# ZephirFXEC/HNanoSolver

Measured on AMD Instinct MI355X. Metric: solver substeps/sec (advect + 50 red-black SOR iterations + project) at N active voxels, higher is better.
Workload: dtype f32

## Files before the change

hnanosolver_amd/csrc/hns_sorblock.hip:

```cpp
#include "hns_device.hpp"
#include "hns_flags.hpp"

namespace hns {


template <int LB, int K>
struct SbGeo {
	static constexpr int H = 2 * K;
	static constexpr int T = 8 * LB + 2 * H;
	static constexpr int C = LB + 2;
	static constexpr int HALF = T / 2;
	static constexpr int ROWS = T * T / 2;
	static constexpr int TC = T - 2;
	static constexpr int HC = TC / 2;
	static constexpr int CROWS = TC * HC;
	static constexpr int RIM = 2 * TC;
	static constexpr int SEC = (CROWS + 63) / 64 * 64;
	static constexpr int NT = 2 * SEC;
	static constexpr int NQ = (HALF + 3) / 4;
	static constexpr int HS4 = 3;
	static constexpr int NCH = T / 4;
	static constexpr int REC = LB == 1 ? 28 : 64;
	static_assert(H % 4 == 0 && H <= 8, "rows must start on a 16-byte piece and stay within the neighbouring leaf");
	static_assert(NQ <= HS4 && NT <= 1024 && RIM <= CROWS, "tile too large");
};

constexpr float kInv6 = 0.166666667f;

template <bool MASKED>
__device__ __forceinline__ float sb_update(float xp, float xm, float yp, float ym, float zp, float zm, float d, float X, float omega, unsigned ok) {
	const float pGS = ((xp + xm + yp + ym + zp + zm) - d) * kInv6;
	const float cand = X + omega * (pGS - X);
	return MASKED ? __uint_as_float(__float_as_uint(cand) & ok) : cand;
}

template <int HALF, int C>
struct SbRow {
	float R[HALF], B[HALF];
	float dR[HALF], dB[HALF];
	unsigned ok[C];
};

template <int LB, int K>
struct SbLds {
	using G = SbGeo<LB, K>;
	static constexpr int NB = G::ROWS * G::HS4, NR = (G::ROWS - 2 * G::HALF) * G::HS4;
	float4 a[2 * (NB + NR)];
	__device__ __forceinline__ float4* arr(int par, int colour) { return a + par * (NB + NR) + (colour ? 0 : NB - G::HALF * G::HS4); }
};

template <int LB, int K, int S, int NS, bool PAR, bool MASKED, class Row>
__device__ __forceinline__ void sb_sweep(Row& r, SbLds<LB, K>& L, const int i, const int b, const int dist, const float omega) {
	using G = SbGeo<LB, K>;
	constexpr int H = G::H, HALF = G::HALF, HS4 = G::HS4;
	constexpr bool red = (S & 1) != 0;
	float(&X)[HALF] = red ? r.R : r.B;
	const float(&Y)[HALF] = red ? r.B : r.R;
	const float(&dX)[HALF] = red ? r.dR : r.dB;
	const float4* LY = L.arr(PAR ? 0 : 1, red ? 1 : 0);
	float4* LX = L.arr(PAR ? 1 : 0, red ? 0 : 1);
	constexpr bool up = red ? PAR : !PAR;
	constexpr int qlo = (S / 2) / 4, qhi = (HALF - S / 2 + 3) / 4;
	constexpr int jlo = 4 * qlo, jhi = 4 * qhi < HALF ? 4 * qhi : HALF;
	if (dist >= S) {
		const float4* pxp = LY + (i + HALF) * HS4;
		const float4* pxm = LY + (i - HALF) * HS4;
		const float4* pyp = LY + (i + b) * HS4;
		const float4* pym = LY + (i + b - 1) * HS4;
		float4 nx[4] = {pxp[qlo], pxm[qlo], pyp[qlo], pym[qlo]};
#pragma unroll
		for (int q = qlo; q < qhi; ++q) {
			const float4 xp4 = nx[0], xm4 = nx[1], yp4 = nx[2], ym4 = nx[3];
			if (q + 1 < qhi) nx[0] = pxp[q + 1], nx[1] = pxm[q + 1], nx[2] = pyp[q + 1], nx[3] = pym[q + 1];
			__builtin_amdgcn_sched_barrier(0);
			const float xp[4] = {xp4.x, xp4.y, xp4.z, xp4.w}, xm[4] = {xm4.x, xm4.y, xm4.z, xm4.w};
			const float yp[4] = {yp4.x, yp4.y, yp4.z, yp4.w}, ym[4] = {ym4.x, ym4.y, ym4.z, ym4.w};
#pragma unroll
			for (int e = 0; e < 4; ++e) {
				const int j = 4 * q + e;
				if (j < jlo || j >= jhi) continue;
				const float below = j > 0 ? Y[j > 0 ? j - 1 : 0] : 0.0f, above = j + 1 < HALF ? Y[j + 1 < HALF ? j + 1 : 0] : 0.0f;
				const float zm = up ? Y[j] : below, zp = up ? above : Y[j];
				const int cz = (2 * j - H + 8) >> 3;
				X[j] = sb_update<MASKED>(xp[e], xm[e], yp[e], ym[e], zp, zm, dX[j], X[j], omega, r.ok[cz]);
			}
			__builtin_amdgcn_sched_barrier(0);
		}
		if (S < NS) {
#pragma unroll
			for (int q = qlo; q < qhi; ++q) {
				const int j = 4 * q;
				LX[i * HS4 + q] = make_float4(X[j], j + 1 < HALF ? X[j + 1 < HALF ? j + 1 : 0] : 0.0f, j + 2 < HALF ? X[j + 2 < HALF ? j + 2 : 0] : 0.0f,
				                              j + 3 < HALF ? X[j + 3 < HALF ? j + 3 : 0] : 0.0f);
			}
		}
	}
	if (S < NS) __syncthreads();
}

template <int LB, int K, int S, int NS, bool PAR, bool MASKED>
struct SbSweeps {
	template <class Row>
	static __device__ __forceinline__ void run(Row& r, SbLds<LB, K>& L, const int i, const int b, const int dist, const float omega) {
		sb_sweep<LB, K, S, NS, PAR, MASKED>(r, L, i, b, dist, omega);
		if constexpr (S < NS) SbSweeps<LB, K, S + 1, NS, PAR, MASKED>::run(r, L, i, b, dist, omega);
	}
};

template <int LB, int K, bool ZERO, bool PAR, int NS>
__device__ __forceinline__ void sb_body(SbLds<LB, K>& L, const int t, const int* __restrict__ recs, const float* __restrict__ div, const float* __restrict__ p_in,
                                        float* __restrict__ p_out, const unsigned field_bytes, const float dx2, const float omega) {
	using G = SbGeo<LB, K>;
	constexpr int H = G::H, T = G::T, C = G::C, HALF = G::HALF, NQ = G::NQ, NCH = G::NCH, HS4 = G::HS4;
	const bool valid = t < G::CROWS;
	const int xq = valid ? t / G::HC : 0;
	const int x = 1 + xq, y = valid ? 1 + 2 * (t - xq * G::HC) + ((x + 1 + (PAR ? 1 : 0)) & 1) : 1;
	const int b = y & 1;
	const int i = x * HALF + (y >> 1);
	const int dist = valid ? min(min(x, T - 1 - x), min(y, T - 1 - y)) : -1;
	const int cx = (x - H + 8) >> 3, cy = (y - H + 8) >> 3;
	const unsigned row_bytes = (unsigned)(((((x - H) & 7) << 3) | ((y - H) & 7)) * 32);
	const int* __restrict__ rec = recs + (size_t)blockIdx.x * G::REC + (LB == 1 ? 1 : 0) + (cx * C + cy) * C;
	unsigned base[C];
	SbRow<HALF, C> r;
#pragma unroll
	for (int cz = 0; cz < C; ++cz) {
		const int id = valid ? rec[cz] : -1;
		r.ok[cz] = id >= 0 ? 0xFFFFFFFFu : 0u;
		base[cz] = (unsigned)id * 2048u + row_bytes;
	}
	const v4i rp = field_rsrc(p_in, field_bytes), rd = field_rsrc(div, field_bytes), ro = field_rsrc(p_out, field_bytes);
	v4f32 pc[NCH], dc[NCH];
#pragma unroll
	for (int j = 0; j < NCH; ++j) {
		const int cz = (4 * j - H + 8) >> 3, zl = (4 * j - H) & 7;
		const unsigned off = base[cz] + (unsigned)(zl * 4);
		dc[j] = hns_buffer_load_v4f32(rd, (int)off, 0, 0);
		if (ZERO) pc[j] = v4f32{0.0f, 0.0f, 0.0f, 0.0f};
		else pc[j] = hns_buffer_load_v4f32(rp, (int)off, 0, 0);
	}
	if (t < G::RIM) {
		const int side = t / G::HC, m = t - side * G::HC;
		const int along = 2 * m + (((side & 1) != 0) == PAR ? 2 : 1);
		const int rx = side == 0 ? 0 : (side == 1 ? T - 1 : along), ry = side == 2 ? 0 : (side == 3 ? T - 1 : along);
		const int rcx = (rx - H + 8) >> 3, rcy = (ry - H + 8) >> 3;
		const unsigned rrow = (unsigned)(((((rx - H) & 7) << 3) | ((ry - H) & 7)) * 32);
		const int* __restrict__ rrec = recs + (size_t)blockIdx.x * G::REC + (LB == 1 ? 1 : 0) + (rcx * C + rcy) * C;
		unsigned rbase[C];
#pragma unroll
		for (int cz = 0; cz < C; ++cz) rbase[cz] = (unsigned)rrec[cz] * 2048u + rrow;
		v4f32 rc[NCH];
#pragma unroll
		for (int j = 0; j < NCH; ++j) rc[j] = ZERO ? v4f32{0.0f, 0.0f, 0.0f, 0.0f} : hns_buffer_load_v4f32(rp, (int)(rbase[(4 * j - H + 8) >> 3] + (unsigned)(((4 * j - H) & 7) * 4)), 0, 0);
		float4* LR = L.arr(PAR ? 1 : 0, 0) + (rx * HALF + (ry >> 1)) * HS4;
		float4* LK = L.arr(PAR ? 1 : 0, 1) + (rx * HALF + (ry >> 1)) * HS4;
		float rr[HALF + 4], rb[HALF + 4];
#pragma unroll
		for (int j = 0; j < NCH; ++j) {
			rr[2 * j] = PAR ? rc[j].y : rc[j].x, rb[2 * j] = PAR ? rc[j].x : rc[j].y;
			rr[2 * j + 1] = PAR ? rc[j].w : rc[j].z, rb[2 * j + 1] = PAR ? rc[j].z : rc[j].w;
		}
#pragma unroll
		for (int q = 0; q < NQ; ++q) {
			if (side >= 2) LR[q] = make_float4(rr[4 * q], rr[4 * q + 1], 4 * q + 2 < HALF ? rr[4 * q + 2] : 0.0f, 4 * q + 3 < HALF ? rr[4 * q + 3] : 0.0f);
			LK[q] = make_float4(rb[4 * q], rb[4 * q + 1], 4 * q + 2 < HALF ? rb[4 * q + 2] : 0.0f, 4 * q + 3 < HALF ? rb[4 * q + 3] : 0.0f);
		}
	}
#pragma unroll
	for (int j = 0; j < NCH; ++j) {
		r.R[2 * j] = PAR ? pc[j].y : pc[j].x, r.B[2 * j] = PAR ? pc[j].x : pc[j].y;
		r.R[2 * j + 1] = PAR ? pc[j].w : pc[j].z, r.B[2 * j + 1] = PAR ? pc[j].z : pc[j].w;
		const float d0 = dc[j].x * dx2, d1 = dc[j].y * dx2, d2 = dc[j].z * dx2, d3 = dc[j].w * dx2;
		r.dR[2 * j] = PAR ? d1 : d0, r.dB[2 * j] = PAR ? d0 : d1;
		r.dR[2 * j + 1] = PAR ? d3 : d2, r.dB[2 * j + 1] = PAR ? d2 : d3;
	}
	if (valid) {
		float4* LR = L.arr(PAR ? 1 : 0, 0) + i * HS4;
		float4* LK = L.arr(PAR ? 1 : 0, 1) + i * HS4;
#pragma unroll
		for (int q = 0; q < NQ; ++q) {
			const int j = 4 * q;
			LR[q] = make_float4(r.R[j], r.R[j + 1], j + 2 < HALF ? r.R[j + 2 < HALF ? j + 2 : 0] : 0.0f, j + 3 < HALF ? r.R[j + 3 < HALF ? j + 3 : 0] : 0.0f);
			LK[q] = make_float4(r.B[j], r.B[j + 1], j + 2 < HALF ? r.B[j + 2 < HALF ? j + 2 : 0] : 0.0f, j + 3 < HALF ? r.B[j + 3 < HALF ? j + 3 : 0] : 0.0f);
		}
	}
	bool mine = true;
#pragma unroll
	for (int cz = 0; cz < C; ++cz) mine = mine && (r.ok[cz] != 0u || !valid);
	const bool all_present = __syncthreads_and(mine) != 0;
	if (all_present)
		SbSweeps<LB, K, 1, NS, PAR, false>::run(r, L, i, b, dist, omega);
	else
		SbSweeps<LB, K, 1, NS, PAR, true>::run(r, L, i, b, dist, omega);
	if (dist >= H) {
#pragma unroll
		for (int j = H / 4; j < NCH - H / 4; ++j) {
			const int cz = (4 * j - H + 8) >> 3, zl = (4 * j - H) & 7;
			v4f32 v;
			v.x = PAR ? r.B[2 * j] : r.R[2 * j], v.y = PAR ? r.R[2 * j] : r.B[2 * j];
			v.z = PAR ? r.B[2 * j + 1] : r.R[2 * j + 1], v.w = PAR ? r.R[2 * j + 1] : r.B[2 * j + 1];
			hns_buffer_store_v4f32(v, ro, (int)(base[cz] + (unsigned)(zl * 4)), 0, 0);
		}
	}
}

template <int C, int HALF>
struct SbLeanRow {
	float dR[HALF], dB[HALF];
	unsigned ok[C];
};

__device__ __forceinline__ void chain_store_piece(const PhaseMirror& m, int leaf, bool mine, int row, int half, v4f32 v) {
	const int e1 = m.first[leaf + 1];
	for (int e = m.first[leaf]; e < e1; ++e) {
		const int2 t = m.entry[e];
		if (!mine) continue;
		const unsigned bits = m.mask ? (m.mask[(size_t)e * 64 + row] >> (4 * half)) & 0xFu : 0xFu;
		float* r = chain_out(m, t.x, 0) + (size_t)t.y * 512 + row * 8 + 4 * half;
		if (bits == 0xFu) {
			store_through(r, chain_v4f{v.x, v.y, v.z, v.w});
		} else if (bits) {
			const float f[4] = {v.x, v.y, v.z, v.w};
#pragma unroll
			for (int z = 0; z < 4; ++z)
				if (bits >> z & 1) store_through(r + z, f[z]);
		}
	}
}

__device__ __forceinline__ void chain_store_piece(const PackMirror& m, int leaf, bool mine, int row, int half, v4f32 v) {
	const int e1 = m.first[leaf + 1];
	for (int e = m.first[leaf]; e < e1; ++e) {
		const int2 t = m.entry[e];
		if (!mine) continue;
		const unsigned byte = m.mask[(size_t)e * 64 + row];
		const unsigned bits = (byte >> (4 * half)) & 0xFu;
		if (!bits) continue;
		float* q = m.msg[t.x] + (size_t)t.y + m.row_pre[(size_t)e * 64 + row] + __popc(byte & ((1u << (4 * half)) - 1u));
		const float f[4] = {v.x, v.y, v.z, v.w};
		int c = 0;
#pragma unroll
		for (int z = 0; z < 4; ++z)
			if (bits >> z & 1) q[c++] = f[z];
	}
}

struct SbLdsXY {
	using G = SbGeo<2, 2>;
	static constexpr int T = G::T, TC = G::TC, HS4 = G::HS4;
	static constexpr int NB = (T * TC + 2 * T) * HS4, NR = TC * TC * HS4;
	float4 a[NB + NR];
	__device__ __forceinline__ float4* black() { return a; }
	__device__ __forceinline__ float4* red() { return a + NB; }
	static __device__ __forceinline__ int brow(int x, int y) { return x * TC + y - 1; }
	static __device__ __forceinline__ int brim(int x, int y) { return T * TC + 2 * x + (y != 0); }
};
static_assert(sizeof(SbLdsXY) == 50880, "the XY form must fit three workgroups per CU (160 KB of LDS)");

template <int S, int NS, bool MASKED, class Row>
__device__ __forceinline__ void sb_sweep_xy(Row& r, SbLdsXY& L, const int bi, const int ypb, const int ymb, const int par, const int dist, const float omega) {
	using G = SbGeo<2, 2>;
	constexpr int H = G::H, HALF = G::HALF, HS4 = G::HS4, NQ = G::NQ, TC = G::TC;
	constexpr bool red = (S & 1) != 0;
	const float(&dX)[HALF] = red ? r.dR : r.dB;
	const bool up = red ? par != 0 : par == 0;
	constexpr int jlo = S / 2, jhi = (G::T - 1 - S) / 2 + 1;
	constexpr int qlo = jlo / 4, qhi = (jhi + 3) / 4;
	if (dist >= S) {
		v4f32* LXo4 = reinterpret_cast<v4f32*>((red ? L.red() + (bi - TC) * HS4 : L.black() + bi * HS4));
		const v4f32* LYo4 = reinterpret_cast<const v4f32*>((red ? L.black() + bi * HS4 : L.red() + (bi - TC) * HS4));
		const float4* LY = red ? L.black() : L.red() - TC * HS4;
		float Y[HALF];
#pragma unroll
		for (int q = 0; q < NQ; ++q) {
			const v4f32 y4 = LYo4[q];
			Y[4 * q] = y4.x, Y[4 * q + 1] = y4.y, Y[4 * q + 2] = y4.z, Y[4 * q + 3] = y4.w;
		}
		const v4f32* pxp = reinterpret_cast<const v4f32*>(LY + (bi + TC) * HS4);
		const v4f32* pxm = reinterpret_cast<const v4f32*>(LY + (bi - TC) * HS4);
		const v4f32* pyp = reinterpret_cast<const v4f32*>(LY + (red ? ypb : bi + 1) * HS4);
		const v4f32* pym = reinterpret_cast<const v4f32*>(LY + (red ? ymb : bi - 1) * HS4);
#pragma unroll
		for (int q = qlo; q < qhi; ++q) {
			v4f32 x4 = LXo4[q], xp4 = pxp[q], xm4 = pxm[q], yp4 = pyp[q], ym4 = pym[q];
			if (4 * q < jlo || 4 * q + 4 > jhi) {
				asm volatile("" : "+v"(x4));
				asm volatile("" : "+v"(xp4));
				asm volatile("" : "+v"(xm4));
				asm volatile("" : "+v"(yp4));
				asm volatile("" : "+v"(ym4));
			}
			float X[4] = {x4.x, x4.y, x4.z, x4.w};
			const float xp[4] = {xp4.x, xp4.y, xp4.z, xp4.w}, xm[4] = {xm4.x, xm4.y, xm4.z, xm4.w}, yp[4] = {yp4.x, yp4.y, yp4.z, yp4.w}, ym[4] = {ym4.x, ym4.y, ym4.z, ym4.w};
#pragma unroll
			for (int e = 0; e < 4; ++e) {
				const int j = 4 * q + e;
				if (j < jlo || j >= jhi) continue;
				const float below = j > 0 ? Y[j > 0 ? j - 1 : 0] : 0.0f, above = j + 1 < HALF ? Y[j + 1 < HALF ? j + 1 : 0] : 0.0f;
				const float zm = up ? Y[j] : below, zp = up ? above : Y[j];
				const int cz = (2 * j - H + 8) >> 3;
				X[e] = sb_update<MASKED>(xp[e], xm[e], yp[e], ym[e], zp, zm, dX[j], X[e], omega, r.ok[cz]);
			}
			v4f32 o4 = v4f32{X[0], X[1], X[2], X[3]};
			if (4 * q < jlo || 4 * q + 4 > jhi) asm volatile("" : "+v"(o4));
			LXo4[q] = o4;
			__builtin_amdgcn_sched_barrier(0);
		}
	}
	if (S < NS) __syncthreads();
}

template <int S, int NS, bool MASKED>
struct SbSweepsXY {
	template <class Row>
	static __device__ __forceinline__ void run(Row& r, SbLdsXY& L, const int bi, const int ypb, const int ymb, const int par, const int dist, const float omega) {
		sb_sweep_xy<S, NS, MASKED>(r, L, bi, ypb, ymb, par, dist, omega);
		if constexpr (S < NS) SbSweepsXY<S + 1, NS, MASKED>::run(r, L, bi, ypb, ymb, par, dist, omega);
	}
};

template <bool ZERO, class M = NoMirror, int NS = 4>
__global__ __attribute__((amdgpu_waves_per_eu(6, 8))) __launch_bounds__((SbGeo<2, 2>::NT)) void k_rbgs_block_xy(const int* __restrict__ recs, const int* __restrict__ any_absent, const float* __restrict__ div, const float* __restrict__ p_in,
                                                                                                                float* __restrict__ p_out, const unsigned field_bytes, const float dx2, const float omega, const M m = M{}) {
	using G = SbGeo<2, 2>;
	constexpr int H = G::H, T = G::T, C = G::C, HALF = G::HALF, NCH = G::NCH, HS4 = G::HS4, TC = G::TC;
	__shared__ SbLdsXY L;
	__shared__ int s_rec[64];
	const int t = threadIdx.x;
	const bool valid = t < TC * TC;
	const int xq = valid ? t / TC : 0;
	const int x = 1 + xq, y = valid ? 1 + t - xq * TC : 1;
	const int par = (x + y) & 1;
	const int bi = SbLdsXY::brow(x, y);
	const int ypb = y == T - 2 ? SbLdsXY::brim(x, T - 1) : bi + 1, ymb = y == 1 ? SbLdsXY::brim(x, 0) : bi - 1;
	const int dist = valid ? min(min(x, T - 1 - x), min(y, T - 1 - y)) : -1;
	const int cx = (x - H + 8) >> 3, cy = (y - H + 8) >> 3;
	const unsigned row_bytes = (unsigned)(((((x - H) & 7) << 3) | ((y - H) & 7)) * 32);
	const int* brec = recs + (size_t)blockIdx.x * G::REC;
	const int rec_word = brec[t & 63];
	const int4 q4 = *reinterpret_cast<const int4*>(brec + (valid ? (cx * C + cy) * C : 0));
	__builtin_amdgcn_sched_barrier(0);
	constexpr int RJ = NCH - 2, NRIM = 4 * TC;
	static_assert(NRIM * RJ <= G::NT && RJ == 4, "one rim piece per thread");
	const bool rim_on = t < NRIM * RJ;
	int rim_b2, rim_zero, rim_par;
	unsigned rim_off;
	bool rim_want;
	int rim_at;
	{
		const int mr = rim_on ? t >> 2 : 0, j = 1 + (t & 3);
		const int side = mr / TC, along = 1 + (mr - side * TC);
		const int rx = side == 0 ? 0 : (side == 1 ? T - 1 : along), ry = side == 2 ? 0 : (side == 3 ? T - 1 : along);
		const int rcx = (rx - H + 8) >> 3, rcy = (ry - H + 8) >> 3, rcz = (4 * j - H + 8) >> 3;
		rim_off = (unsigned)(((((rx - H) & 7) << 3) | ((ry - H) & 7)) * 32 + ((4 * j - H) & 7) * 4);
		rim_b2 = (side >= 2 ? SbLdsXY::brim(rx, ry) : SbLdsXY::brow(rx, ry)) * HS4 * 2 + j;
		rim_par = (rx + ry) & 1;
		rim_want = !ZERO && rim_on && along >= H && along < T - H;
		rim_at = rim_want ? (rcx * C + rcy) * C + rcz : 0;
		rim_zero = j == 1 ? -1 : (j == RJ ? 1 : 0);
	}
	const int rim_id = brec[rim_at];
	const int meta_word = any_absent[blockIdx.x];
	__builtin_amdgcn_sched_barrier(0);
	SbLeanRow<C, HALF> r;
	unsigned base[C], dbase[C];
	constexpr unsigned kBeyond = 0xFFFFF000u;
	{
		const int ids[C] = {valid ? q4.x : -1, valid ? q4.y : -1, valid ? q4.z : -1, valid ? q4.w : -1};
		const int e = max(0, max(H - x, x - (T - 1 - H))) + max(0, max(H - y, y - (T - 1 - H)));
#pragma unroll
		for (int cz = 0; cz < C; ++cz) {
			r.ok[cz] = ids[cz] >= 0 ? 0xFFFFFFFFu : 0u;
			const unsigned b = (unsigned)ids[cz] * 2048u + row_bytes;
			const bool end = cz == 0 || cz == C - 1;
			base[cz] = e > (end ? H - 1 : H) ? kBeyond : b;
			dbase[cz] = e > (end ? H - 2 : H - 1) ? kBeyond : b;
		}
	}
	int chain_leaf = 0x7fffffff;
	if constexpr (!std::is_same<M, NoMirror>::value) {
		if (__builtin_amdgcn_readfirstlane(meta_word) & 2) chain_leaf = 0;
		chain_begin(m, chain_leaf);
		__syncthreads();
	}
	const v4i rp = field_rsrc(p_in, field_bytes), rd = field_rsrc(div, field_bytes), ro = field_rsrc(p_out, field_bytes);
	v4f32 pc[NCH], dc[NCH], rimv;
#pragma unroll
	for (int j = 0; j < NCH; ++j) pc[j] = ZERO ? v4f32{0.0f, 0.0f, 0.0f, 0.0f} : hns_buffer_load_v4f32(rp, (int)(base[(4 * j - H + 8) >> 3] + (unsigned)(((4 * j - H) & 7) * 4)), 0, 0);
	__builtin_amdgcn_sched_barrier(0);
	rimv = ZERO ? v4f32{0.0f, 0.0f, 0.0f, 0.0f} : hns_buffer_load_v4f32(rp, (int)((unsigned)(rim_want ? rim_id : -1) * 2048u + rim_off), 0, 0);
#pragma unroll
	for (int j = 0; j < NCH; ++j) dc[j] = hns_buffer_load_v4f32(rd, (int)(dbase[(4 * j - H + 8) >> 3] + (unsigned)(((4 * j - H) & 7) * 4)), 0, 0);
	if (t < 64) s_rec[t] = rec_word;
	if (rim_on) {
		float2* LK = reinterpret_cast<float2*>(L.black()) + rim_b2;
		*LK = rim_par ? make_float2(rimv.x, rimv.z) : make_float2(rimv.y, rimv.w);
		if (rim_zero) LK[rim_zero] = make_float2(0.0f, 0.0f);
	}
	if (valid) {
		float4* LE = par ? L.black() + bi * HS4 : L.red() + (bi - TC) * HS4;
		float4* LO = par ? L.red() + (bi - TC) * HS4 : L.black() + bi * HS4;
#pragma unroll
		for (int q = 0; q < G::NQ; ++q) {
			const v4f32 u = pc[2 * q], v = pc[2 * q + 1];
			LE[q] = make_float4(u.x, u.z, v.x, v.z);
			LO[q] = make_float4(u.y, u.w, v.y, v.w);
		}
	}
	const int meta = __builtin_amdgcn_readfirstlane(meta_word);
#pragma unroll
	for (int j = 0; j < NCH; ++j) {
		const float d0 = dc[j].x * dx2, d1 = dc[j].y * dx2, d2 = dc[j].z * dx2, d3 = dc[j].w * dx2;
		r.dR[2 * j] = par ? d1 : d0, r.dB[2 * j] = par ? d0 : d1;
		r.dR[2 * j + 1] = par ? d3 : d2, r.dB[2 * j + 1] = par ? d2 : d3;
	}
	__syncthreads();
	if ((meta & 1) == 0)
		SbSweepsXY<1, NS, false>::run(r, L, bi, ypb, ymb, par, dist, omega);
	else
		SbSweepsXY<1, NS, true>::run(r, L, bi, ypb, ymb, par, dist, omega);
	__syncthreads();
	{
		int mirror_id[8] = {-1, -1, -1, -1, -1, -1, -1, -1};
		if constexpr (!std::is_same<M, NoMirror>::value) {
			if (meta & 2) {
#pragma unroll
				for (int c = 0; c < 8; ++c)
					mirror_id[c] = (meta >> (8 + c)) & 1 ? __builtin_amdgcn_readfirstlane(s_rec[((1 + (c >> 2)) * C + 1 + ((c >> 1) & 1)) * C + 1 + (c & 1)]) : -1;
			}
		}
		const float2* B2 = reinterpret_cast<const float2*>(L.black());
		const float2* R2 = reinterpret_cast<const float2*>(L.red());
#pragma unroll
		for (int n = 0; n < 2; ++n) {
			const int pq = t + n * G::NT;
			const int jz = pq & 1, yy = (pq >> 1) & 15, czb = (pq >> 5) & 1, xx = pq >> 6;
			const int sx = xx + H, sy = yy + H, j = H / 4 + 2 * czb + jz;
			const int sp = (sx + sy) & 1;
			const int sb = SbLdsXY::brow(sx, sy);
			const float2 rr = R2[(sb - TC) * HS4 * 2 + j], bb = B2[sb * HS4 * 2 + j];
			const int cell = (((xx >> 3) << 1) | (yy >> 3)) << 1 | czb;
			const int id = (meta >> (8 + cell)) & 1 ? s_rec[((1 + (xx >> 3)) * C + 1 + (yy >> 3)) * C + 1 + czb] : -1;
			v4f32 v;
			v.x = sp ? bb.x : rr.x, v.y = sp ? rr.x : bb.x, v.z = sp ? bb.y : rr.y, v.w = sp ? rr.y : bb.y;
			hns_buffer_store_v4f32(v, ro, (int)((unsigned)id * 2048u + (unsigned)((((xx & 7) << 3) | (yy & 7)) * 32 + jz * 16)), 0, 0);
			if constexpr (!std::is_same<M, NoMirror>::value) {
				if (meta & 2) {
#pragma unroll
					for (int cc = 0; cc < 4; ++cc) {
						const int c = 4 * n + cc;
						const int lc = mirror_id[c];
						if (lc < 0 || lc >= m.n_boundary) continue;
						chain_store_piece(m, lc, c == cell, ((xx & 7) << 3) | (yy & 7), jz, v);
					}
				}
			}
		}
	}
	if constexpr (!std::is_same<M, NoMirror>::value) chain_end(m, chain_leaf);
}

template <int LB, int K, bool ZERO, int NS = 2 * K>
__global__ __launch_bounds__((SbGeo<LB, K>::NT)) void k_rbgs_block(const int* __restrict__ recs, const float* __restrict__ div, const float* __restrict__ p_in, float* __restrict__ p_out,
                                                                   const unsigned field_bytes, const float dx2, const float omega) {
	using G = SbGeo<LB, K>;
	static_assert(LB == 1, "rows in registers: one-leaf blocks (16^3 blocks are swept by k_rbgs_block_xy)");
	__shared__ SbLds<LB, K> L;
	const int t = threadIdx.x;
	if (__builtin_amdgcn_readfirstlane(t >= G::SEC))
		sb_body<LB, K, ZERO, true, NS>(L, t - G::SEC, recs, div, p_in, p_out, field_bytes, dx2, omega);
	else
		sb_body<LB, K, ZERO, false, NS>(L, t, recs, div, p_in, p_out, field_bytes, dx2, omega);
}


__global__ __launch_bounds__(256) void k_sb_leader(GridDev g, int first, int count, int* __restrict__ flag) {
	const int l = blockIdx.x * 256 + threadIdx.x;
	if (l >= g.n_leaves) return;
	int lead = (l >= first && l < first + count) ? 1 : 0;
	if (lead) {
		const int4 o = g.origins[l];
		const int bx = o.x & ~15, by = o.y & ~15, bz = o.z & ~15;
		for (int c = 0; c < 8; ++c) {
			const int q = d_find_leaf(g, bx + 8 * (c >> 2), by + 8 * ((c >> 1) & 1), bz + 8 * (c & 1));
			if (q >= first && q < l) lead = 0;
		}
	}
	flag[l] = lead;
}

__global__ __launch_bounds__(1024) void k_sb_compact(const int* __restrict__ flag, int n, int* __restrict__ leaders, int* __restrict__ total, int n_head) {
	__shared__ int s_part[1024];
	const int per = (n + 1023) / 1024;
	const int lo = threadIdx.x * per, hi = min(n, lo + per);
	int sum = 0;
	for (int i = lo; i < hi; ++i) sum += flag[i];
	s_part[threadIdx.x] = sum;
	__syncthreads();
	for (int d = 1; d < 1024; d <<= 1) {
		const int v = threadIdx.x >= d ? s_part[threadIdx.x - d] : 0;
		__syncthreads();
		s_part[threadIdx.x] += v;
		__syncthreads();
	}
	int run = s_part[threadIdx.x] - sum;
	for (int i = lo; i < hi; ++i) {
		if (i == n_head) total[1] = run;
		if (flag[i]) leaders[run++] = i;
	}
	if (threadIdx.x == 1023) {
		total[0] = s_part[1023];
		if (n_head >= n) total[1] = s_part[1023];
	}
}

__global__ __launch_bounds__(256) void k_sb_table(GridDev g, const int* __restrict__ leaders, int n_blocks, int seg, int pre, int first, int count, int n_boundary, int* __restrict__ tab) {
	const int64_t i = (int64_t)blockIdx.x * 256 + threadIdx.x;
	if (i >= (int64_t)n_blocks * 64) return;
	const int b = (int)(i >> 6), c = (int)(i & 63);
	const int4 o = g.origins[leaders[sched_leaf(b, n_blocks, seg, pre)]];
	const int cx = c >> 4, cy = (c >> 2) & 3, cz = c & 3;
	const int64_t x = (int64_t)(o.x & ~15) + 8 * (cx - 1), y = (int64_t)(o.y & ~15) + 8 * (cy - 1), z = (int64_t)(o.z & ~15) + 8 * (cz - 1);
	int leaf = -1;
	if (x >= INT32_MIN && x <= INT32_MAX && y >= INT32_MIN && y <= INT32_MAX && z >= INT32_MIN && z <= INT32_MAX) leaf = d_find_leaf(g, (int)x, (int)y, (int)z);
	tab[i] = leaf;
	int* meta = tab + (int64_t)n_blocks * 64 + b;
	if (leaf < 0) atomicOr(meta, 1);
	const bool inner = ((cx - 1) | (cy - 1) | (cz - 1)) >= 0 && cx <= 2 && cy <= 2 && cz <= 2;
	if (inner && leaf >= first && leaf < first + count) atomicOr(meta, (1 << (8 + ((((cx - 1) << 1) | (cy - 1)) << 1 | (cz - 1)))) | (leaf < n_boundary ? 2 : 0));
}

}

using namespace hns;

void hns_grid_retire_blocks(hns_grid* g);

int hns_grid_build_blocks(hns_grid* g) {
	std::lock_guard<std::mutex> lock(g->build_mutex);
	const int seg = 0;
	if (g->sb_built && g->sb_seg == seg && g->sb_first == g->first_active && g->sb_count == g->n_active) return HNS_OK;
	if (g->d_sb_tab) {
		if (g->sb_retired.size() >= 64) {
			HNS_HIP(hipDeviceSynchronize());
			hns_grid_retire_blocks(g);
		}
		g->sb_retired.emplace_back(g->d_sb_tab, g->sb_bytes);
	}
	g->d_sb_tab = nullptr;
	g->sb_bytes = 0;
	g->n_sb = 0;
	g->sb_built = true;
	g->sb_seg = seg;
	g->sb_first = g->first_active, g->sb_count = g->n_active;
	const int n = (int)g->topo.n_leaves;
	if (n == 0 || g->n_active == 0 || !g->d_scratch) return HNS_OK;
	int* flag = (int*)g->d_scratch;
	int* leaders = flag + n;
	int* total = leaders + n;
	GridDev gd = g->dev();
	const int first = (int)g->first_active, count = (int)g->n_active;
	const int n_boundary = g->chain_boundary ? first + (int)std::min<uint64_t>(g->chain_boundary, g->n_active) : 0;
	hipStream_t st = nullptr;
	HNS_HIP(hipStreamCreateWithFlags(&st, hipStreamNonBlocking));
	struct Drop {
		hipStream_t s;
		~Drop() { (void)hipStreamDestroy(s); }
	} drop{st};
	hipLaunchKernelGGL(k_sb_leader, dim3((n + 255) / 256), dim3(256), 0, st, gd, first, count, flag);
	hipLaunchKernelGGL(k_sb_compact, dim3(1), dim3(1024), 0, st, (const int*)flag, n, leaders, total, n_boundary);
	int tot[2] = {0, 0};
	HNS_HIP(hipMemcpyAsync(tot, total, 2 * sizeof(int), hipMemcpyDeviceToHost, st));
	HNS_HIP(hipStreamSynchronize(st));
	const int nb = tot[0];
	if (nb <= 0) return fail(HNS_ERR_RUNTIME, "hns_grid_build_blocks: no block leader found");
	if (int rc = hns_arena_get(sizeof(int) * 65 * (size_t)nb, g->device, &g->d_sb_tab, &g->sb_bytes)) return rc;
	HNS_HIP(hipMemsetAsync((int*)g->d_sb_tab + (size_t)nb * 64, 0, sizeof(int) * (size_t)nb, st));
	const int pre = (n_boundary && g->sched_prefix) ? (std::min(tot[1], nb) & ~7) : 0;
	hipLaunchKernelGGL(k_sb_table, dim3((unsigned)(((int64_t)nb * 64 + 255) / 256)), dim3(256), 0, st, gd, (const int*)leaders, nb, seg, pre, first, count, n_boundary, (int*)g->d_sb_tab);
	HNS_HIP(hipStreamSynchronize(st));
	g->n_sb = (uint64_t)nb;
	return HNS_OK;
}

void hns_grid_retire_blocks(hns_grid* g) {
	for (auto& t : g->sb_retired) hns_arena_put(t.first, t.second, g->device);
	g->sb_retired.clear();
}

static int hns_rbgs_block_shape(hns_grid* g, int* k_max) {
	*k_max = 0;
	if (g->n_active == 0 || g->topo.n_leaves > 2000000) return 0;
	int lb = options().sor_block_lb.load();
	if (lb == 0) lb = g->n_active <= 600 ? 1 : 2;
	if (lb != 1 && lb != 2) return 0;
	if (lb == 1 && !g->d_blk) return 0;
	if (lb == 2 && (hns_grid_build_blocks(g) != HNS_OK || g->n_sb == 0)) return 0;
	*k_max = (lb == 1 && g->n_active <= 300) ? 4 : 2;
	return lb;
}

static SorSchedule blocked_schedule(hns_grid* g, int iterations) {
	int k_max = 0;
	const int lb = iterations >= 1 ? hns_rbgs_block_shape(g, &k_max) : 0;
	return sor_schedule(lb, k_max, iterations);
}

SorSchedule hns_rbgs_schedule(hns_grid* g, int iterations) {
	return options().rbgs.load() == kRbgsColor ? sor_schedule(0, 0, iterations) : blocked_schedule(g, iterations);
}

static bool two_in_one_xy_launch(hns_grid* g) {
	const SorSchedule s = blocked_schedule(g, 2);
	return s.one_blocked_launch() && s.lb == 2;
}

template <int K, int NS>
static void launch_leaf_blocks(hns_grid* g, bool src_is_zero, const float* div, const float* src, float* dst, float dx2, float omega, hipStream_t st) {
	const unsigned bytes = (unsigned)((size_t)g->topo.n_leaves * 2048u);
	auto* kernel = src_is_zero ? k_rbgs_block<1, K, true, NS> : k_rbgs_block<1, K, false, NS>;
	hipLaunchKernelGGL(kernel, dim3((unsigned)g->n_active), dim3(SbGeo<1, K>::NT), 0, st, (const int*)g->d_blk, div, src, dst, bytes, dx2, omega);
}

enum class XYLaunch { done, no_records, bad_iterations };
template <class M>
static XYLaunch launch_xy_blocks(hns_grid* g, int iterations, bool src_is_zero, const float* div, const float* src, float* dst, float dx2, float omega, const M& m, hipStream_t st) {
	const int* tab;
	uint64_t n_sb;
	{
		std::lock_guard<std::mutex> lock(g->build_mutex);
		tab = (const int*)g->d_sb_tab, n_sb = g->n_sb;
	}
	if (!tab || !n_sb) return XYLaunch::no_records;
	if (iterations != 1 && iterations != 2) return XYLaunch::bad_iterations;
	const unsigned bytes = (unsigned)((size_t)g->topo.n_leaves * 2048u);
	auto* kernel = iterations == 2 ? (src_is_zero ? k_rbgs_block_xy<true, M, 4> : k_rbgs_block_xy<false, M, 4>) : (src_is_zero ? k_rbgs_block_xy<true, M, 2> : k_rbgs_block_xy<false, M, 2>);
	hipLaunchKernelGGL(kernel, dim3((unsigned)n_sb), dim3(SbGeo<2, 2>::NT), 0, st, tab, tab + (size_t)n_sb * 64, div, src, dst, bytes, dx2, omega, m);
	return XYLaunch::done;
}

int hns_rbgs_block_launch(hns_grid* g, int lb, int k, bool src_is_zero, const float* div, const float* src, float* dst, float dx2, float omega, void* stream) {
	hipStream_t st = (hipStream_t)stream;
	if (lb == 1 && k == 2) launch_leaf_blocks<2, 4>(g, src_is_zero, div, src, dst, dx2, omega, st);
	else if (lb == 1 && k == 4) launch_leaf_blocks<4, 8>(g, src_is_zero, div, src, dst, dx2, omega, st);
	else if (lb == 1 && k == 1) launch_leaf_blocks<2, 2>(g, src_is_zero, div, src, dst, dx2, omega, st);
	else {
		const XYLaunch r = lb == 2 ? launch_xy_blocks(g, k, src_is_zero, div, src, dst, dx2, omega, NoMirror{}, st) : XYLaunch::bad_iterations;
		if (r == XYLaunch::no_records) return fail(HNS_ERR_RUNTIME, "hns_rbgs_block_launch: no block records");
		if (r != XYLaunch::done) return fail(HNS_ERR_INVALID_ARGUMENT, "hns_rbgs_block_launch: unsupported block shape");
	}
	return HNS_OK;
}

extern "C" __attribute__((visibility("hidden"))) bool hns_rbgs_block_packable(hns_grid* g) { return g && g->n_active && two_in_one_xy_launch(g); }

extern "C" __attribute__((visibility("hidden"))) int hns_rbgs_block_pack_launch(hns_grid* g, const float* div, const float* src, float* dst, float dx, float omega, bool src_is_zero,
                                                                                 const hns::PackMirror* m, void* stream, bool* done, int iterations) {
	*done = false;
	if (!hns_rbgs_block_packable(g)) return HNS_OK;
	if (int rc = hns_grid_build_blocks(g)) return rc;
	const XYLaunch r = launch_xy_blocks(g, iterations, src_is_zero, div, src, dst, dx * dx , omega, *m, (hipStream_t)stream);
	if (r == XYLaunch::bad_iterations) return fail(HNS_ERR_INVALID_ARGUMENT, "hns_rbgs_block_pack_launch: one or two iterations per launch");
	*done = r == XYLaunch::done;
	return HNS_OK;
}

extern "C" __attribute__((visibility("hidden"))) int hns_rbgs_block_mirror_launch(hns_grid* g, const float* div, const float* src, float* dst, float dx, float omega, bool src_is_zero,
                                                                                   const hns::PhaseMirror* m, void* stream, int iterations) {
	if (!two_in_one_xy_launch(g)) return fail(HNS_ERR_RUNTIME, "hns_rbgs_block_mirror_launch: this launch range is not swept in 16^3 blocks");
	const XYLaunch r = launch_xy_blocks(g, iterations, src_is_zero, div, src, dst, dx * dx , omega, *m, (hipStream_t)stream);
	if (r == XYLaunch::no_records) return fail(HNS_ERR_RUNTIME, "hns_rbgs_block_mirror_launch: no block records");
	if (r == XYLaunch::bad_iterations) return fail(HNS_ERR_INVALID_ARGUMENT, "hns_rbgs_block_mirror_launch: one or two iterations per launch");
	return HNS_OK;
}
```

Baseline: 644.8.

## Remap SOR block threads into shell-ordered rows so inactive sweeps skip whole waves

Replaces the row-major thread-to-row mapping in the XY red-black block kernel with a shell layout. Interior 16-row strips, edge strips and corner quads are each packed into 16-lane runs, so rows that drop out of later sweeps sit together in whole waves. The per-sweep activity test moves from a square distance-to-boundary check to the summed per-axis excess `e`, which also skips corner rows the dependency cone does not need. The y ordering within strips is rotated per x, apparently to spread LDS bank access. The costs are more complex index arithmetic and possibly less coalesced global loads for the permuted rows.

```diff
diff --git a/hnanosolver_amd/csrc/hns_sorblock.hip b/hnanosolver_amd/csrc/hns_sorblock.hip
--- a/hnanosolver_amd/csrc/hns_sorblock.hip
+++ b/hnanosolver_amd/csrc/hns_sorblock.hip
@@ -257,8 +257,37 @@
 };
 static_assert(sizeof(SbLdsXY) == 50880, "the XY form must fit three workgroups per CU (160 KB of LDS)");
 
+struct SbShells {
+	using G = SbGeo<2, 2>;
+	static constexpr int H = G::H, T = G::T;
+	static constexpr int STRIPS = 16 * (T - 2 * H) + 6 * 16, QUADS = 384;
+	static_assert(H == 4 && T == 24 && STRIPS + 32 == QUADS && QUADS + 4 * 2 * 16 == G::NT, "16-lane runs, whole waves, 512 threads");
+	static __device__ __forceinline__ bool row(const int t, int& x, int& y, int& e) {
+		if (t < STRIPS) {
+			const int run = t >> 4, s = (run - 16) >> 1;
+			x = run < 16 ? H + run : (run & 1 ? T - H + s : H - 1 - s);
+			y = H + (((t & 15) - 6 * x + 8) & 15);
+			e = run < 16 ? 0 : s + 1;
+			return true;
+		}
+		if (t < QUADS) {
+			const int c = t - STRIPS;
+			const int ex = (0x231211 >> (4 * (c >> 2) & 31)) & 15, ey = (0x213121 >> (4 * (c >> 2) & 31)) & 15;
+			const bool v = c < 24;
+			x = v ? (c & 1 ? T - 1 - H + ex : H - ex) : 1, y = v ? (c & 2 ? T - 1 - H + ey : H - ey) : 1, e = v ? ex + ey : 2 * H;
+			return v;
+		}
+		const int u = t - QUADS, i = u & 3, q = (u >> 2) & 7, h = u >> 5;
+		const bool v = i != 0;
+		x = H + 8 * (h & 1) + ((0x76452310 >> (4 * q)) & 7);
+		y = v ? (h & 2 ? T - 1 - H + i : i) : 1;
+		e = v ? (h & 2 ? i : H - i) : 2 * H;
+		return v;
+	}
+};
+
 template <int S, int NS, bool MASKED, class Row>
-__device__ __forceinline__ void sb_sweep_xy(Row& r, SbLdsXY& L, const int bi, const int ypb, const int ymb, const int par, const int dist, const float omega) {
+__device__ __forceinline__ void sb_sweep_xy(Row& r, SbLdsXY& L, const int bi, const int ypb, const int ymb, const int par, const int e, const float omega) {
 	using G = SbGeo<2, 2>;
 	constexpr int H = G::H, HALF = G::HALF, HS4 = G::HS4, NQ = G::NQ, TC = G::TC;
 	constexpr bool red = (S & 1) != 0;
@@ -266,7 +295,7 @@
 	const bool up = red ? par != 0 : par == 0;
 	constexpr int jlo = S / 2, jhi = (G::T - 1 - S) / 2 + 1;
 	constexpr int qlo = jlo / 4, qhi = (jhi + 3) / 4;
-	if (dist >= S) {
+	if (e <= NS - S) {
 		v4f32* LXo4 = reinterpret_cast<v4f32*>((red ? L.red() + (bi - TC) * HS4 : L.black() + bi * HS4));
 		const v4f32* LYo4 = reinterpret_cast<const v4f32*>((red ? L.black() + bi * HS4 : L.red() + (bi - TC) * HS4));
 		const float4* LY = red ? L.black() : L.red() - TC * HS4;
@@ -313,9 +342,9 @@
 template <int S, int NS, bool MASKED>
 struct SbSweepsXY {
 	template <class Row>
-	static __device__ __forceinline__ void run(Row& r, SbLdsXY& L, const int bi, const int ypb, const int ymb, const int par, const int dist, const float omega) {
-		sb_sweep_xy<S, NS, MASKED>(r, L, bi, ypb, ymb, par, dist, omega);
-		if constexpr (S < NS) SbSweepsXY<S + 1, NS, MASKED>::run(r, L, bi, ypb, ymb, par, dist, omega);
+	static __device__ __forceinline__ void run(Row& r, SbLdsXY& L, const int bi, const int ypb, const int ymb, const int par, const int e, const float omega) {
+		sb_sweep_xy<S, NS, MASKED>(r, L, bi, ypb, ymb, par, e, omega);
+		if constexpr (S < NS) SbSweepsXY<S + 1, NS, MASKED>::run(r, L, bi, ypb, ymb, par, e, omega);
 	}
 };
 
@@ -327,13 +356,11 @@
 	__shared__ SbLdsXY L;
 	__shared__ int s_rec[64];
 	const int t = threadIdx.x;
-	const bool valid = t < TC * TC;
-	const int xq = valid ? t / TC : 0;
-	const int x = 1 + xq, y = valid ? 1 + t - xq * TC : 1;
+	int x, y, e;
+	const bool valid = SbShells::row(t, x, y, e);
 	const int par = (x + y) & 1;
 	const int bi = SbLdsXY::brow(x, y);
 	const int ypb = y == T - 2 ? SbLdsXY::brim(x, T - 1) : bi + 1, ymb = y == 1 ? SbLdsXY::brim(x, 0) : bi - 1;
-	const int dist = valid ? min(min(x, T - 1 - x), min(y, T - 1 - y)) : -1;
 	const int cx = (x - H + 8) >> 3, cy = (y - H + 8) >> 3;
 	const unsigned row_bytes = (unsigned)(((((x - H) & 7) << 3) | ((y - H) & 7)) * 32);
 	const int* brec = recs + (size_t)blockIdx.x * G::REC;
@@ -367,7 +394,6 @@
 	constexpr unsigned kBeyond = 0xFFFFF000u;
 	{
 		const int ids[C] = {valid ? q4.x : -1, valid ? q4.y : -1, valid ? q4.z : -1, valid ? q4.w : -1};
-		const int e = max(0, max(H - x, x - (T - 1 - H))) + max(0, max(H - y, y - (T - 1 - H)));
 #pragma unroll
 		for (int cz = 0; cz < C; ++cz) {
 			r.ok[cz] = ids[cz] >= 0 ? 0xFFFFFFFFu : 0u;
@@ -416,9 +442,9 @@
 	}
 	__syncthreads();
 	if ((meta & 1) == 0)
-		SbSweepsXY<1, NS, false>::run(r, L, bi, ypb, ymb, par, dist, omega);
+		SbSweepsXY<1, NS, false>::run(r, L, bi, ypb, ymb, par, e, omega);
 	else
-		SbSweepsXY<1, NS, true>::run(r, L, bi, ypb, ymb, par, dist, omega);
+		SbSweepsXY<1, NS, true>::run(r, L, bi, ypb, ymb, par, e, omega);
 	__syncthreads();
 	{
 		int mirror_id[8] = {-1, -1, -1, -1, -1, -1, -1, -1};
```

After: 651.7 (median of 6 runs). 1.01x the previous value.
